# DCMMC/halo2-scaffold

Measured on AMD Instinct MI355X. Metric: create_proof() wall-clock + MSM G1-adds/s at k=20 standard_plonk, 1/2/4/8 GPU, higher is better.
Workload: dtype u32 (254-bit Montgomery integers as 9 x 29-bit limbs, 64-bit multiply-accumulate); 1 GPU; standard_plonk hot-path replay k=20: 11 MSM(2^20) + 6 iNTT(2^20) + 6 coset-NTT(2^21) + 1 coset-iNTT(2^21); k=20, scalar_distribution=uniform, msm_window_bits=17, msm_windows=15, msm_buckets=65536, parallelism=single-gpu, deployment=one process, one GPU, combine=none (single GPU)

## Files before the change

### halo2-scaffold_amd/csrc/h2mi_msm.hip

```cpp

#include <algorithm>
#include <map>
#include <type_traits>
#include <vector>

#include "g1.cuh"
#include "g1_29.cuh"
#include "g1_29_quad.cuh"
#include "h2mi_internal.h"
#include "scan.cuh"

namespace h2 {

constexpr uint32_t S0_MAX = 128;
constexpr uint32_t S1 = 8;
constexpr uint32_t FG_NARROW = 8;
constexpr uint32_t FG_WIDE = 2;
constexpr size_t SHIFT_MIN_N = 4096;
constexpr uint32_t HOT_MIN = 64;
constexpr uint32_t HOT_MIN_WIDE = 8;

constexpr uint32_t ACCUM_RESIDENT_CHUNKS = 256 * 2 * 256;
__host__ __device__ inline uint32_t accum_rounds(uint32_t entries) {
  const uint32_t per_round = S0_MAX * ACCUM_RESIDENT_CHUNKS;
// ... 20 lines not shown
  hipError_t wait(hipStream_t s) const { return hipStreamWaitEvent(s, ev, 0); }
  hipError_t wait_if_pending(hipStream_t s) const { return pending ? wait(s) : hipSuccess; }
  hipError_t wait_if_ever(hipStream_t s) const { return ever ? wait(s) : hipSuccess; }
};

struct Slot {
  uint32_t* vals[2] = {nullptr, nullptr};
  uint8_t* bkeys = nullptr;
  uint32_t* bincnt = nullptr;
  uint32_t* binbase = nullptr;
  uint32_t* binseg = nullptr;
  uint32_t* tile_live = nullptr;
  uint32_t* off = nullptr;
  uint32_t* s0_dev = nullptr;
  uint32_t* np[2] = {nullptr, nullptr};
  uint32_t* toff[2] = {nullptr, nullptr};
  uint8_t* part[2] = {nullptr, nullptr};
  uint8_t* dense = nullptr;
  uint8_t *dense2 = nullptr, *vsum = nullptr;
  uint32_t* tseg[2] = {nullptr, nullptr};
  uint8_t* rc = nullptr;
  uint8_t* g = nullptr;
  uint64_t* stats = nullptr;
  fe* shift = nullptr;
  Stage input_ready;
  Stage head, accum, tail;
  hipStream_t last_stream = nullptr;
  bool tail_deferred = false;
  void* d_out = nullptr;
  uint32_t tasks1 = 0;
  uint8_t* sdig = nullptr;
  uint8_t* spart = nullptr;
  uint32_t* scnt = nullptr;
  bool small_deferred = false;
  uint32_t small_n = 0;

  hipError_t create_events() {
    for (Stage* st : {&input_ready, &head, &accum, &tail})
      if (hipError_t e = st->create()) return e;
    return hipSuccess;
  }
  void destroy_events() {
    for (Stage* st : {&input_ready, &head, &accum, &tail}) st->destroy();
  }
  void clear_pending() { tail.pending = accum.pending = head.pending = false; }
  hipError_t reduction_launched(hipStream_t t) {
    const hipError_t e = tail.record(t);
    if (e == hipSuccess) tail_deferred = small_deferred = false;
    return e;
  }
};
constexpr int NSLOT = 8;

struct Bases {
  int dev = 0;
  size_t n = 0;
  size_t stride = 0;
  bool has_sum = false;
  uint32_t c = 0, W = 0, nb = 0, logNl = 0, logNh = 0;
  uint32_t seg_log = 0;
  uint8_t* table = nullptr;
  uint8_t* host_stage = nullptr;
  uint32_t lb = 0, nbins = 0;
  Slot slot[NSLOT];
  int nslot = NSLOT;
  int next_slot = 0, last_slot = 0;
  uint32_t max_tasks0 = 0, max_tasks1 = 0;
  bool small = false;
  uint32_t sc = 0, sW = 0, slanes = 0, sr = 0, sG = 0;
  uint8_t* stable = nullptr;
  uint32_t since_join = 0;
  bool last_small = false;
};

static std::map<uint64_t, Bases*> g_bases;
struct AdHoc {
  size_t n;
  uint64_t fp[2];
  uint64_t handle;
  uint64_t last_use;
};
static std::vector<AdHoc> g_adhoc;
static uint64_t g_adhoc_clock = 0, g_adhoc_builds = 0;
constexpr size_t ADHOC_MAX = 4;
static bool g_canonical = false;
constexpr size_t SMALL_STREAM_N = (size_t)1 << 13;
constexpr uint32_t SMALL_STREAM_AFTER = 4;
static uint64_t g_next_handle = 1;

__global__ void __launch_bounds__(256) k_msm_table_first(const uint8_t* bases, uint8_t* table0, size_t n) {
  size_t i = (size_t)blockIdx.x * blockDim.x + threadIdx.x;
  if (i >= n) return;
  affine p = affine_load(bases + i * 64);
  if (!affine_is_identity(p)) {
    f29 x, y;
    affine_to_f29(p, x, y);
    f29_pack(x, p.x.v);
    f29_pack(y, p.y.v);
  }
  affine_store(table0 + i * 64, p);
}
__global__ void __launch_bounds__(256) k_msm_table_next(const uint8_t* prev, uint8_t* next, size_t n, uint32_t c) {
  size_t i = (size_t)blockIdx.x * blockDim.x + threadIdx.x;
  if (i >= n) return;
  affine p = affine_load(prev + i * 64);
  if (affine_is_identity(p)) {
    affine_store(next + i * 64, p);
    return;
  }
  xyzz29 acc = xyzz29_dbl_affine(f29_unpack(p.x.v), f29_unpack(p.y.v));
  for (uint32_t k = 1; k < c; k++) acc = xyzz29_dbl(acc);
  f29 x, y;
  xyzz29_to_affine(acc, x, y);
  affine q;
  f29_pack(x, q.x.v);
  f29_pack(y, q.y.v);
  affine_store(next + i * 64, q);
}

__global__ void __launch_bounds__(64) k_msm_table_sum_point(const uint8_t* sum_jac, uint8_t* table, size_t stride, size_t n, uint32_t W, uint32_t c) {
  const uint32_t w = threadIdx.x;
  if (w >= W) return;
  const xyzz29 b = xyzz29_from_jac(jac_load(sum_jac));
  affine out;
  out.x = fe_zero();
  out.y = fe_zero();
  if (!xyzz29_is_identity(b)) {
    f29 x, y;
    xyzz29_to_affine(b, x, y);
    if (w) {
      xyzz29 acc = xyzz29_dbl_affine(x, y);
      for (uint32_t k = 1; k < c * w; k++) acc = xyzz29_dbl(acc);
      xyzz29_to_affine(acc, x, y);
    }
    f29_pack(x, out.x.v);
    f29_pack(y, out.y.v);
  }
  affine_store(table + ((size_t)w * stride + n) * 64, out);
}
__global__ void __launch_bounds__(256) k_msm_fill_one(fe* out, size_t n) {
  size_t i = (size_t)blockIdx.x * blockDim.x + threadIdx.x;
  if (i < n) fe_store(&out[i], fe_one<FrP>());
}

constexpr uint32_t P1_TS = 768;
constexpr uint32_t NBINS_MAX = 512;
constexpr uint32_t WIDE_MIN_C = 18, WIDE_MAX_C = 20, MAT_LOG = 16;
constexpr uint32_t WIDE_BIN_BITS = 9;
template <bool WIDE>
__device__ __forceinline__ uint32_t bin_of(uint32_t bucket, uint32_t lb) { return WIDE ? (bucket & ((1u << WIDE_BIN_BITS) - 1)) : (bucket >> lb); }
template <bool WIDE>
__device__ __forceinline__ uint32_t key_of(uint32_t bucket, uint32_t mask) { return WIDE ? (bucket >> WIDE_BIN_BITS) : (bucket & mask); }
constexpr uint32_t P2_THREADS = 512, P2_PER = 16, P2_CH = P2_THREADS * P2_PER;

template <uint32_t CT, class F>
__device__ __forceinline__ void for_each_digit(const fe& s, uint32_t c_rt, uint32_t W_rt, F&& f) {
  const uint32_t c = CT ? CT : c_rt;
  const uint32_t W = CT ? (255 + CT - 1) / CT : W_rt;
  uint32_t carry = 0;
  const uint32_t half = 1u << (c - 1);
#pragma unroll
  for (uint32_t w = 0; w < W; w++) {
    uint32_t bit = w * c;
    uint32_t limb = bit >> 5, sh = bit & 31;
    uint32_t raw = 0;
    if (limb < 8) {
      uint64_t two = s.v[limb];
      if (limb + 1 < 8) two |= (uint64_t)s.v[limb + 1] << 32;
      raw = (uint32_t)(two >> sh) & ((1u << c) - 1);
    }
    uint32_t d = raw + carry;
    uint32_t mag = d, neg = 0;
    carry = 0;
    if (d > half) {
      mag = (1u << c) - d;
      neg = 1;
      carry = 1;
    }
    if (mag) f(w, mag - 1, neg);
  }
}


__device__ __forceinline__ void msm_pick_shift_body(const fe* scalars, size_t n, fe* shift_out) {
  __shared__ fe smp[64];
  const uint32_t lane = threadIdx.x;
  size_t idx = (n / 64) * lane + n / 128;
  if (idx >= n) idx = n - 1;
  const fe v = fe_load(&scalars[idx]);
  smp[lane] = v;
  __syncthreads();
  uint32_t same = 0;
  for (uint32_t j = 0; j < 64; j++) same += fe_eq(v, smp[j]) ? 1u : 0u;
  const uint64_t winners = __ballot(same >= 40);
  if (lane == 0) fe_store(shift_out, winners ? smp[__ffsll((unsigned long long)winners) - 1] : fe_zero());
}
__global__ void __launch_bounds__(64) k_msm_pick_shift(const fe* scalars, size_t n, fe* shift_out) { msm_pick_shift_body(scalars, n, shift_out); }
__device__ __forceinline__ fe msm_scalar(const fe* scalars, size_t i, size_t n, const fe* shift) {
  fe x;
  if (!shift) {
    x = fe_load(&scalars[i]);
  } else {
    const fe v = fe_load(shift);
    x = i < n ? fe_sub<FrP>(fe_load(&scalars[i]), v) : v;
  }
  if (fe_is_zero(x)) return x;
  f29 c = f29_zero();
  c.v[0] = 32;
  fe o;
  f29_pack(f29_reduce_canonical<Fr29>(f29_mul<Fr29>(f29_unpack(x.v), c)), o.v);
  return o;
}

template <uint32_t CT>
__device__ __forceinline__ void msm_bin_count_body(const fe* scalars, size_t n, const fe* shift, uint32_t c, uint32_t W, uint32_t lb, uint32_t nbins,
                                                   uint32_t ntiles, uint32_t* cnt_out, uint32_t* tile_live) {
  __shared__ uint32_t cnt[NBINS_MAX];
  __shared__ uint32_t any_live;
  const uint32_t tid = threadIdx.x;
  if (tid < NBINS_MAX) cnt[tid] = 0;
  if (tid == 0) any_live = 0;
  __syncthreads();
  size_t i = (size_t)blockIdx.x * P1_TS + tid;
  if (i < n + (shift ? 1 : 0)) {
    fe s = msm_scalar(scalars, i, n, shift);
    if (!fe_is_zero(s)) {
      any_live = 1;
      for_each_digit<CT>(s, c, W, [&](uint32_t, uint32_t bucket, uint32_t) { atomicAdd(&cnt[bin_of<(CT >= WIDE_MIN_C)>(bucket, lb)], 1u); });
    }
  }
  __syncthreads();
  if (tid == 0) tile_live[blockIdx.x] = any_live;
  if (tid < nbins) cnt_out[(size_t)tid * ntiles + blockIdx.x] = cnt[tid];
  if (blockIdx.x == 0 && tid == 0) cnt_out[(size_t)nbins * ntiles] = 0;
}
template <uint32_t CT>
__global__ void __launch_bounds__(P1_TS) k_msm_bin_count(const fe* scalars, size_t n, const fe* shift, uint32_t c, uint32_t W, uint32_t lb,
                                                         uint32_t nbins, uint32_t ntiles, uint32_t* cnt_out, uint32_t* tile_live) {
  msm_bin_count_body<CT>(scalars, n, shift, c, W, lb, nbins, ntiles, cnt_out, tile_live);
}

extern __shared__ uint4 h2_msm_smem[];

template <uint32_t CT>
__device__ __forceinline__ void msm_bin_scatter_body(const fe* scalars, size_t n, const fe* shift, size_t n_reg, uint32_t c, uint32_t W, uint32_t lb,
                                                     uint32_t nbins, uint32_t ntiles, const uint32_t* base, uint32_t* vals_out, void* keys_out_,
                                                     const uint32_t* tile_live) {
  constexpr bool WIDE = CT >= WIDE_MIN_C;
  if (!tile_live[blockIdx.x]) return;
  __shared__ uint32_t cnt[NBINS_MAX], lstart[NBINS_MAX + 1], wsum[NBINS_MAX / 64];
  uint32_t* stage_val = reinterpret_cast<uint32_t*>(h2_msm_smem);
  uint16_t* stage_key = reinterpret_cast<uint16_t*>(stage_val + P1_TS * W);
  const uint32_t tid = threadIdx.x, lane = tid & 63, wave = tid >> 6, tile = blockIdx.x;
  uint32_t gb = 0;
  if (tid < NBINS_MAX) {
    cnt[tid] = 0;
    gb = tid < nbins ? base[(size_t)tid * ntiles + tile] : 0;
  }
  __syncthreads();
  size_t i = (size_t)tile * P1_TS + tid;
  fe s;
  const bool live = i < n + (shift ? 1 : 0);
  constexpr uint32_t WK = CT ? (255 + CT - 1) / CT : 1;
  uint32_t ent[WK], rk[WK];
#pragma unroll
  for (uint32_t w = 0; w < WK; w++) ent[w] = 0xFFFFFFFFu;
  bool live_nz = false;
  if (live) {
    s = msm_scalar(scalars, i, n, shift);
    live_nz = !fe_is_zero(s);
  }
  if (live_nz) {
    for_each_digit<CT>(s, c, W, [&](uint32_t w, uint32_t bucket, uint32_t neg) {
      uint32_t r = atomicAdd(&cnt[bin_of<WIDE>(bucket, lb)], 1u);
      if (CT) {
        ent[w] = bucket | (neg << 31);
        rk[w] = r;
      }
    });
  }
  __syncthreads();
  uint32_t v = 0, inc = 0;
  if (tid < NBINS_MAX) {
    v = cnt[tid];
    inc = wave_incl_scan(v);
    if (lane == 63) wsum[wave] = inc;
  }
  __syncthreads();
  if (tid < NBINS_MAX) {
    uint32_t add = 0;
    for (uint32_t j = 0; j < wave; j++) add += wsum[j];
    lstart[tid] = add + inc - v;
    cnt[tid] = add + inc - v;
    if (tid == NBINS_MAX - 1) lstart[NBINS_MAX] = add + inc;
  }
  __syncthreads();
  const uint32_t mask = (1u << lb) - 1;
  if (CT) {
#pragma unroll
    for (uint32_t w = 0; w < WK; w++)
      if (ent[w] != 0xFFFFFFFFu) {
        const uint32_t bucket = ent[w] & 0x7FFFFFFFu;
        const uint32_t pos = lstart[bin_of<WIDE>(bucket, lb)] + rk[w];
        stage_val[pos] = (ent[w] & 0x80000000u) | (uint32_t)((size_t)w * n_reg + i);
        stage_key[pos] = (uint16_t)(WIDE ? key_of<true>(bucket, mask) : bucket);
      }
  } else if (live_nz) {
    for_each_digit<CT>(s, c, W, [&](uint32_t w, uint32_t bucket, uint32_t neg) {
      uint32_t pos = atomicAdd(&cnt[bucket >> lb], 1u);
      stage_val[pos] = (neg << 31) | (uint32_t)((size_t)w * n_reg + i);
      stage_key[pos] = (uint16_t)bucket;
    });
  }
  __syncthreads();
  if (tid < NBINS_MAX) cnt[tid] = gb - lstart[tid];
  __syncthreads();
  const uint32_t total = lstart[NBINS_MAX];
  if (WIDE) {
    uint16_t* keys_out = reinterpret_cast<uint16_t*>(keys_out_);
    for (uint32_t p = tid; p < total; p += P1_TS) {
      uint32_t lo = 0, hi = NBINS_MAX;
      while (hi - lo > 1) {
        const uint32_t mid = (lo + hi) >> 1;
        if (lstart[mid] <= p) lo = mid;
        else hi = mid;
      }
      const uint32_t dst = p + cnt[lo];
      vals_out[dst] = stage_val[p];
      keys_out[dst] = stage_key[p];
    }
  } else {
    uint8_t* keys_out = reinterpret_cast<uint8_t*>(keys_out_);
    for (uint32_t p = tid; p < total; p += P1_TS) {
      const uint32_t key = stage_key[p];
      const uint32_t dst = p + cnt[key >> lb];
      vals_out[dst] = stage_val[p];
      keys_out[dst] = (uint8_t)(key & mask);
    }
  }
}
template <uint32_t CT>
__global__ void __launch_bounds__(P1_TS) k_msm_bin_scatter(const fe* scalars, size_t n, const fe* shift, size_t n_reg, uint32_t c, uint32_t W,
                                                           uint32_t lb, uint32_t nbins, uint32_t ntiles, const uint32_t* base, uint32_t* vals_out,
                                                           void* keys_out_, const uint32_t* tile_live) {
  msm_bin_scatter_body<CT>(scalars, n, shift, n_reg, c, W, lb, nbins, ntiles, base, vals_out, keys_out_, tile_live);
}

constexpr uint32_t NQ_MAX = 128;
__device__ __forceinline__ void msm_bin_sort_body(const uint8_t* keys_in, const uint32_t* vals_in, const uint32_t* base, uint32_t ntiles, uint32_t nbins,
                                                  uint32_t lb, uint32_t s0_fixed, uint32_t nb, uint32_t* vals_out, uint32_t* off, uint32_t* np0,
                                                  uint32_t* np1, uint32_t* s0_out) {
  __shared__ uint32_t wh[P2_THREADS / 64][NQ_MAX];
  __shared__ uint32_t run[NQ_MAX], ccnt[NQ_MAX], cstart[NQ_MAX], carry64;
  __shared__ uint32_t stage[P2_CH];
  __shared__ uint8_t stage_q[P2_CH];
  const uint32_t tid = threadIdx.x, wave = tid >> 6, bin = blockIdx.x;
  const uint32_t start = base[(size_t)bin * ntiles], end = base[(size_t)(bin + 1) * ntiles];
  const uint32_t nq = 1u << lb;
  const uint32_t entries = base[(size_t)nbins * ntiles];
  const uint32_t s0 = s0_fixed ? s0_fixed : accum_chunk_len(entries);
  for (uint32_t j = tid; j < (P2_THREADS / 64) * NQ_MAX; j += P2_THREADS) (&wh[0][0])[j] = 0;
  __syncthreads();
  for (uint32_t j = (start & ~15u) + tid * 16; j < end; j += P2_THREADS * 16) {
    const uint4 kk = *reinterpret_cast<const uint4*>(keys_in + j);
    const uint32_t w4[4] = {kk.x, kk.y, kk.z, kk.w};
#pragma unroll
    for (uint32_t t = 0; t < 16; t++) {
      const uint32_t idx = j + t;
      if (idx >= start && idx < end) atomicAdd(&wh[wave][(w4[t >> 2] >> (8 * (t & 3))) & (NQ_MAX - 1)], 1u);
    }
  }
  __syncthreads();
  uint32_t tot = 0, inc = 0;
  if (tid < NQ_MAX) {
#pragma unroll
    for (uint32_t w = 0; w < P2_THREADS / 64; w++) tot += wh[w][tid];
    inc = wave_incl_scan(tot);
    if (tid == 63) carry64 = inc;
  }
  __syncthreads();
  if (tid < NQ_MAX) {
    const uint32_t ex = inc - tot + (tid >= 64 ? carry64 : 0);
    run[tid] = start + ex;
    ccnt[tid] = 0;
    if (tid < nq) {
      const uint32_t b = (bin << lb) + tid;
      const uint32_t o = start + ex;
      off[b] = o;
      uint32_t f0 = tot ? 1u + (o + tot - 1) / s0 - o / s0 : 0u;
      np0[b] = f0;
      np1[b] = (f0 + S1 - 1) / S1;
    }
    if (bin == 0 && tid == 0) {
      off[nb] = entries;
      np0[nb] = 0;
      np1[nb] = 0;
      *s0_out = s0;
    }
  }
  __syncthreads();
  for (uint32_t cs = start; cs < end; cs += P2_CH) {
    const uint32_t m = min(P2_CH, end - cs);
    uint32_t q[P2_PER], v[P2_PER], r[P2_PER];
#pragma unroll
    for (uint32_t k = 0; k < P2_PER; k++) {
      const uint32_t p = k * P2_THREADS + tid;
      if (p < m) {
        q[k] = keys_in[cs + p] & (NQ_MAX - 1);
        v[k] = vals_in[cs + p];
      }
    }
#pragma unroll
    for (uint32_t k = 0; k < P2_PER; k++)
      if (k * P2_THREADS + tid < m) r[k] = atomicAdd(&ccnt[q[k]], 1u);
    __syncthreads();
    uint32_t cn = 0, cinc = 0;
    if (tid < NQ_MAX) {
      cn = ccnt[tid];
      cinc = wave_incl_scan(cn);
      if (tid == 63) carry64 = cinc;
    }
    __syncthreads();
    if (tid < NQ_MAX) cstart[tid] = cinc - cn + (tid >= 64 ? carry64 : 0);
    __syncthreads();
#pragma unroll
    for (uint32_t k = 0; k < P2_PER; k++)
      if (k * P2_THREADS + tid < m) {
        const uint32_t pos = cstart[q[k]] + r[k];
        stage[pos] = v[k];
        stage_q[pos] = (uint8_t)q[k];
      }
    __syncthreads();
    for (uint32_t p = tid; p < m; p += P2_THREADS) {
      const uint32_t qq = stage_q[p];
      vals_out[run[qq] + (p - cstart[qq])] = stage[p];
    }
    __syncthreads();
    if (tid < NQ_MAX) {
      run[tid] += ccnt[tid];
      ccnt[tid] = 0;
    }
    __syncthreads();
  }
}
__global__ void __launch_bounds__(P2_THREADS) k_msm_bin_sort(const uint8_t* keys_in, const uint32_t* vals_in, const uint32_t* base, uint32_t ntiles,
                                                             uint32_t nbins, uint32_t lb, uint32_t s0_fixed, uint32_t nb, uint32_t* vals_out,
                                                             uint32_t* off, uint32_t* np0, uint32_t* np1, uint32_t* s0_out) {
  msm_bin_sort_body(keys_in, vals_in, base, ntiles, nbins, lb, s0_fixed, nb, vals_out, off, np0, np1, s0_out);
}

constexpr uint32_t NQW = 1024, P2W_PER = 12, P2W_CH = P2_THREADS * P2W_PER;
__device__ __forceinline__ void block_excl_scan_1024(const uint32_t* in, uint32_t* out, uint32_t* wtot ) {
  const uint32_t tid = threadIdx.x, lane = tid & 63, wave = tid >> 6;
  const uint32_t a = in[2 * tid], b = in[2 * tid + 1];
  const uint32_t inc = wave_incl_scan(a + b);
  if (lane == 63) wtot[wave] = inc;
  __syncthreads();
  uint32_t add = 0;
  for (uint32_t w = 0; w < wave; w++) add += wtot[w];
  const uint32_t ex = add + inc - (a + b);
  __syncthreads();
  out[2 * tid] = ex;
  out[2 * tid + 1] = ex + a;
}
__global__ void __launch_bounds__(P2_THREADS) k_msm_bin_sort_wide(const uint16_t* keys_in, const uint32_t* vals_in, const uint32_t* base,
                                                                  uint32_t ntiles, uint32_t nbins, uint32_t lb, uint32_t s0_fixed, uint32_t nb,
                                                                  uint32_t* vals_out, uint32_t* off, uint32_t* np0, uint32_t* np1, uint32_t* s0_out) {
  __shared__ uint32_t hist[NQW], run[NQW], ccnt[NQW], cstart[NQW], wtot[P2_THREADS / 64];
  __shared__ uint32_t stage[P2W_CH];
  __shared__ uint16_t stage_q[P2W_CH];
  const uint32_t tid = threadIdx.x, bin = blockIdx.x;
  const uint32_t start = base[(size_t)bin * ntiles], end = base[(size_t)(bin + 1) * ntiles];
  const uint32_t nq = 1u << lb;
  const uint32_t entries = base[(size_t)nbins * ntiles];
  const uint32_t s0 = s0_fixed ? s0_fixed : accum_chunk_len(entries);
  for (uint32_t j = tid; j < NQW; j += P2_THREADS) {
    hist[j] = 0;
    ccnt[j] = 0;
  }
  __syncthreads();
  for (uint32_t j = (start & ~7u) + tid * 8; j < end; j += P2_THREADS * 8) {
    const uint4 kk = *reinterpret_cast<const uint4*>(keys_in + j);
    const uint32_t w4[4] = {kk.x, kk.y, kk.z, kk.w};
#pragma unroll
    for (uint32_t t = 0; t < 8; t++) {
      const uint32_t idx = j + t;
      if (idx >= start && idx < end) atomicAdd(&hist[(w4[t >> 1] >> (16 * (t & 1))) & (NQW - 1)], 1u);
    }
  }
  __syncthreads();
  block_excl_scan_1024(hist, cstart, wtot);
  __syncthreads();
  for (uint32_t q = tid; q < NQW; q += P2_THREADS) {
    const uint32_t ex = cstart[q], tot = hist[q];
    run[q] = start + ex;
    if (q < nq) {
      const uint32_t b = (bin << lb) + q;
      const uint32_t o = start + ex;
      off[b] = o;
      const uint32_t f0 = tot ? 1u + (o + tot - 1) / s0 - o / s0 : 0u;
      np0[b] = f0;
      np1[b] = (f0 + S1 - 1) / S1;
    }
  }
  if (bin == 0 && tid == 0) {
    off[nb] = entries;
    np0[nb] = 0;
    np1[nb] = 0;
    *s0_out = s0;
  }
  __syncthreads();
  for (uint32_t cs = start; cs < end; cs += P2W_CH) {
    const uint32_t m = min(P2W_CH, end - cs);
    uint32_t q[P2W_PER], v[P2W_PER], r[P2W_PER];
#pragma unroll
    for (uint32_t k = 0; k < P2W_PER; k++) {
      const uint32_t p = k * P2_THREADS + tid;
      if (p < m) {
        q[k] = keys_in[cs + p] & (NQW - 1);
        v[k] = vals_in[cs + p];
      }
    }
#pragma unroll
    for (uint32_t k = 0; k < P2W_PER; k++)
      if (k * P2_THREADS + tid < m) r[k] = atomicAdd(&ccnt[q[k]], 1u);
    __syncthreads();
    block_excl_scan_1024(ccnt, cstart, wtot);
    __syncthreads();
#pragma unroll
    for (uint32_t k = 0; k < P2W_PER; k++)
      if (k * P2_THREADS + tid < m) {
        const uint32_t pos = cstart[q[k]] + r[k];
        stage[pos] = v[k];
        stage_q[pos] = (uint16_t)q[k];
      }
    __syncthreads();
    for (uint32_t p = tid; p < m; p += P2_THREADS) {
      const uint32_t qq = stage_q[p];
      vals_out[run[qq] + (p - cstart[qq])] = stage[p];
    }
    __syncthreads();
    for (uint32_t qi = tid; qi < NQW; qi += P2_THREADS) {
      run[qi] += ccnt[qi];
      ccnt[qi] = 0;
    }
    __syncthreads();
  }
}

constexpr uint32_t PART_BYTES = 144;
__device__ __forceinline__ xyzz29 part_load(const uint8_t* p) {
  const uint4* q = reinterpret_cast<const uint4*>(p);
  uint32_t w[36];
#pragma unroll
  for (int i = 0; i < 9; i++) {
    uint4 v = q[i];
    w[4 * i] = v.x; w[4 * i + 1] = v.y; w[4 * i + 2] = v.z; w[4 * i + 3] = v.w;
  }
  xyzz29 r;
#pragma unroll
  for (int i = 0; i < 9; i++) { r.x.v[i] = w[i]; r.y.v[i] = w[9 + i]; r.zz.v[i] = w[18 + i]; r.zzz.v[i] = w[27 + i]; }
  return r;
}
__device__ __forceinline__ void part_store(uint8_t* p, const xyzz29& a) {
  uint32_t w[36];
#pragma unroll
  for (int i = 0; i < 9; i++) { w[i] = a.x.v[i]; w[9 + i] = a.y.v[i]; w[18 + i] = a.zz.v[i]; w[27 + i] = a.zzz.v[i]; }
  uint4* q = reinterpret_cast<uint4*>(p);
#pragma unroll
  for (int i = 0; i < 9; i++) q[i] = make_uint4(w[4 * i], w[4 * i + 1], w[4 * i + 2], w[4 * i + 3]);
}

__device__ __forceinline__ uint32_t find_bucket(const uint32_t* toff, uint32_t nb, uint32_t t) {
  uint32_t lo = 0, hi = nb;
  while (hi - lo > 1) {
    uint32_t mid = (lo + hi) >> 1;
    if (toff[mid] <= t) lo = mid;
    else hi = mid;
  }
  return lo;
}

typedef affine tab_entry;
__device__ __forceinline__ tab_entry tab_load(const uint8_t* table, uint32_t i) { return affine_load(table + (size_t)i * 64); }
__device__ __forceinline__ bool tab_is_identity(const tab_entry& p) { return affine_is_identity(p); }
__device__ __forceinline__ f29 tab_x(const tab_entry& p) { return f29_unpack(p.x.v); }
__device__ __forceinline__ f29 tab_y(const tab_entry& p) { return f29_unpack(p.y.v); }

__device__ __forceinline__ void msm_accum_body(const uint32_t* entries, const uint32_t* off, const uint32_t* toff, uint32_t nb, const uint32_t* s0_dev,
                                               const uint8_t* table, uint8_t* part) {
  const uint32_t t = blockIdx.x * blockDim.x + threadIdx.x;
  const uint32_t total = off[nb];
  const uint32_t s0 = *s0_dev;
  if ((uint64_t)t * s0 >= total) return;
  const uint32_t start = t * s0;
  const uint32_t end = min(start + s0, total);
  uint32_t b = find_bucket(off, nb, start);
  uint32_t pidx = toff[b] + (t - off[b] / s0);
  uint32_t bend = off[b + 1];
  xyzz29 acc = xyzz29_identity();
  uint32_t e = entries[start];
  tab_entry nxt = tab_load(table, e & 0x7fffffffu);
  uint32_t nneg = e >> 31;
  for (uint32_t k = start; k < end; k++) {
    if (k == bend) {
      part_store(part + (size_t)pidx * PART_BYTES, acc);
      pidx++;
      acc = xyzz29_identity();
      do {
        b++;
        bend = off[b + 1];
      } while (bend == k);
    }
    tab_entry p = nxt;
    uint32_t neg = nneg;
    if (k + 1 < end) {
      e = entries[k + 1];
      nxt = tab_load(table, e & 0x7fffffffu);
      nneg = e >> 31;
    }
    if (tab_is_identity(p)) continue;
    f29 x2 = tab_x(p);
    f29 y2 = tab_y(p);
    if (neg) y2 = f29_sub(f29_zero(), y2, Fq29::K2);
    xyzz29_madd(acc, x2, y2);
  }
  part_store(part + (size_t)pidx * PART_BYTES, acc);
}
__global__ void __launch_bounds__(256) k_msm_accum(const uint32_t* entries, const uint32_t* off, const uint32_t* toff, uint32_t nb,
                                                    const uint32_t* s0_dev, const uint8_t* table, uint8_t* part) {
  msm_accum_body(entries, off, toff, nb, s0_dev, table, part);
}

constexpr size_t ACCUM_LDS = 56000;

constexpr uint32_t HEAD_BATCH = 4;
struct HeadDesc {
  const fe* scalars;
  fe* shift;
  uint32_t *bincnt, *tile_live, *binseg, *binbase, *vals0, *vals1, *off, *np0, *np1, *toff0, *toff1, *s0_dev;
  void* bkeys;
  uint8_t* part0;
};
struct HeadBatch {
  HeadDesc d[HEAD_BATCH];
};
__global__ void __launch_bounds__(64) k_msm_pick_shift_b(const HeadBatch hb, size_t n) {
  const HeadDesc& d = hb.d[blockIdx.y];
  msm_pick_shift_body(d.scalars, n, d.shift);
}
template <uint32_t CT>
__global__ void __launch_bounds__(P1_TS) k_msm_bin_count_b(const HeadBatch hb, size_t n, uint32_t c, uint32_t W, uint32_t lb, uint32_t nbins,
                                                           uint32_t ntiles) {
  const HeadDesc& d = hb.d[blockIdx.y];
  msm_bin_count_body<CT>(d.scalars, n, d.shift, c, W, lb, nbins, ntiles, d.bincnt, d.tile_live);
}
template <uint32_t CT>
__global__ void __launch_bounds__(P1_TS) k_msm_bin_scatter_b(const HeadBatch hb, size_t n, size_t n_reg, uint32_t c, uint32_t W, uint32_t lb,
                                                             uint32_t nbins, uint32_t ntiles) {
  const HeadDesc& d = hb.d[blockIdx.y];
  msm_bin_scatter_body<CT>(d.scalars, n, d.shift, n_reg, c, W, lb, nbins, ntiles, d.binbase, d.vals0, d.bkeys, d.tile_live);
}
__global__ void __launch_bounds__(P2_THREADS) k_msm_bin_sort_b(const HeadBatch hb, uint32_t ntiles, uint32_t nbins, uint32_t lb, uint32_t s0_fixed,
                                                               uint32_t nb) {
  const HeadDesc& d = hb.d[blockIdx.y];
  msm_bin_sort_body((const uint8_t*)d.bkeys, d.vals0, d.binbase, ntiles, nbins, lb, s0_fixed, nb, d.vals1, d.off, d.np0, d.np1, d.s0_dev);
}
__global__ void __launch_bounds__(256) k_msm_accum_b(const HeadBatch hb, uint32_t nb, const uint8_t* table) {
  const HeadDesc& d = hb.d[blockIdx.y];
  msm_accum_body(d.vals1, d.off, d.toff0, nb, d.s0_dev, table, d.part0);
}
__global__ void __launch_bounds__(1024) k_scan_segsum_bins_b(const HeadBatch hb, uint32_t m) {
  const HeadDesc& d = hb.d[blockIdx.y];
  scan_segsum_body<SCAN_SEG_BINS>(d.bincnt, m, d.binseg);
}
__global__ void __launch_bounds__(1024) k_scan_seg_bins_b(const HeadBatch hb, uint32_t m) {
  const HeadDesc& d = hb.d[blockIdx.y];
  scan_seg_body<SCAN_SEG_BINS>(d.bincnt, d.binbase, m, d.binseg);
}
__global__ void __launch_bounds__(1024) k_scan_seg_tasks_b(const HeadBatch hb, uint32_t m) {
  const HeadDesc& d = hb.d[blockIdx.z];
  scan_seg_body<SCAN_SEG_TASKS>(blockIdx.y ? d.np1 : d.np0, blockIdx.y ? d.toff1 : d.toff0, m, nullptr);
}

constexpr uint32_t TAIL_BATCH = 8;
struct TailDesc {
  const uint8_t* part0;
  const uint32_t *toff0, *np0, *toff1, *np1, *off;
  uint8_t *part1, *dense, *rc, *g, *out;
  uint64_t* stats;
  uint32_t nb, logNh, logNl, canonical;
  const uint8_t* mat;
  uint8_t *dense2, *vsum;
  uint32_t seg_log;
  uint32_t hot_min;
  uint32_t no_fold;
};
struct TailBatch {
  TailDesc d[TAIL_BATCH];
};

constexpr uint32_t TAIL_THREADS = 512;

template <bool QUAD>
__global__ void __launch_bounds__(256) k_msm_fold(const TailBatch tb) {
  const TailDesc& d = tb.d[blockIdx.y];
  if (d.no_fold) return;
  const uint32_t nb = d.nb;
  const uint32_t *toff_out = d.toff1, *toff_in = d.toff0, *np_in = d.np0;
  const uint32_t t = (blockIdx.x * blockDim.x + threadIdx.x) >> (QUAD ? 2 : 0);
  if (t >= toff_out[nb]) return;
  uint32_t b = find_bucket(toff_out, nb, t);
  uint32_t j = t - toff_out[b];
  const uint32_t m = np_in[b], np = toff_out[b + 1] - toff_out[b];
  const uint32_t q = m / np, r = m - q * np;
  uint32_t start = toff_in[b] + j * q + min(j, r);
  uint32_t len = q + (j < r ? 1u : 0u);
  xyzz29 acc = part_load(d.part0 + (size_t)start * PART_BYTES);
  for (uint32_t k = 1; k < len; k++) {
    xyzz29 p = part_load(d.part0 + (size_t)(start + k) * PART_BYTES);
    if (QUAD) acc = xyzz29_add_quad(acc, p);
    else xyzz29_add(acc, p);
  }
  if (!QUAD || (threadIdx.x & 3u) == 0) part_store(d.part1 + (size_t)t * PART_BYTES, acc);
}

__device__ __forceinline__ xyzz29 shfl_down_xyzz(const xyzz29& a, uint32_t delta) {
  xyzz29 r;
#pragma unroll
  for (int i = 0; i < 9; i++) {
    r.x.v[i] = __shfl_down(a.x.v[i], delta);
    r.y.v[i] = __shfl_down(a.y.v[i], delta);
    r.zz.v[i] = __shfl_down(a.zz.v[i], delta);
    r.zzz.v[i] = __shfl_down(a.zzz.v[i], delta);
  }
  return r;
}
__device__ __forceinline__ void msm_finish_hot_body(const TailDesc& d, uint32_t bx);
template <bool QUAD, uint32_t FG>
__global__ void __launch_bounds__(256) k_msm_finish(const TailBatch tb, uint32_t hot_blocks) {
  const TailDesc& d = tb.d[blockIdx.y];
  if (blockIdx.x < hot_blocks) {
    msm_finish_hot_body(d, blockIdx.x);
    return;
  }
  const uint32_t bx = blockIdx.x - hot_blocks;
  const uint32_t nb = d.nb;
  constexpr uint32_t LW = QUAD ? 2 : 0;
  const uint32_t worker = (bx * blockDim.x + threadIdx.x) >> LW;
  const uint32_t b = worker / FG, l = worker % FG;
  if ((bx * blockDim.x >> LW) / FG >= nb) return;
  xyzz29 acc = xyzz29_identity();
  bool hot = false;
  if (b < nb) {
    uint32_t cnt = d.np1[b], s = d.toff1[b];
    hot = cnt > d.hot_min;
    if (hot) cnt = 0;
    for (uint32_t k = l; k < cnt; k += FG) {
      xyzz29 p = part_load(d.part1 + (size_t)(s + k) * PART_BYTES);
      if (QUAD) acc = xyzz29_add_quad(acc, p);
      else xyzz29_add(acc, p);
    }
  }
  for (uint32_t dd = FG / 2; dd > 0; dd >>= 1) {
    xyzz29 o = shfl_down_xyzz(acc, dd << LW);
    if (l < dd) {
      if (QUAD) acc = xyzz29_add_quad(acc, o);
      else xyzz29_add(acc, o);
    }
  }
  if (b < nb && !hot && l == 0 && (!QUAD || (threadIdx.x & 3u) == 0)) part_store(d.dense + (size_t)b * PART_BYTES, acc);
}

__device__ __forceinline__ void block_tree_sum(xyzz29* lds, uint32_t count_pow2) {
  const uint32_t quad = threadIdx.x >> 2, nquads = blockDim.x >> 2;
  for (uint32_t s = count_pow2 >> 1; s > 0; s >>= 1) {
    for (uint32_t g = quad; g < s; g += nquads) {
      xyzz29 r = xyzz29_add_quad(lds[g], lds[g + s]);
      if ((threadIdx.x & 3u) == 0) lds[g] = r;
    }
    __syncthreads();
  }
}

__device__ __forceinline__ void msm_finish_hot_body(const TailDesc& d, uint32_t bx) {
  __shared__ uint32_t hot_list[256], nhot;
  const uint32_t tid = threadIdx.x, quad = tid >> 2;
  const uint32_t b = bx * 256 + tid;
  if (tid == 0) nhot = 0;
  __syncthreads();
  if (b < d.nb && d.np1[b] > d.hot_min) hot_list[atomicAdd(&nhot, 1u)] = b;
  __syncthreads();
  const uint32_t n_hot = nhot;
  xyzz29* lds = reinterpret_cast<xyzz29*>(h2_msm_smem);
  for (uint32_t h = 0; h < n_hot; h++) {
    const uint32_t hb = hot_list[h];
    const uint32_t cnt = d.np1[hb], s = d.toff1[hb];
    xyzz29 acc = xyzz29_identity();
    for (uint32_t k = quad; k < cnt; k += 64) acc = xyzz29_add_quad(acc, part_load(d.part1 + (size_t)(s + k) * PART_BYTES));
    if ((tid & 3u) == 0) lds[quad] = acc;
    __syncthreads();
    block_tree_sum(lds, 64);
    if (tid == 0) part_store(d.dense + (size_t)hb * PART_BYTES, lds[0]);
    __syncthreads();
  }
}

__global__ void __launch_bounds__(256) k_msm_seg(const TailBatch tb) {
  const TailDesc& d = tb.d[blockIdx.y];
  if (!d.seg_log) return;
  const uint32_t L = 1u << d.seg_log, s = (blockIdx.x * blockDim.x + threadIdx.x) >> 2;
  if (s >= (d.nb >> d.seg_log)) return;
  const uint32_t lb = MAT_LOG + d.seg_log - WIDE_BIN_BITS;
  xyzz29 T = xyzz29_identity(), V = xyzz29_identity();
  for (uint32_t j = 0; j < L; j++) {
    const uint32_t b = s * L + j, bp = ((b & ((1u << WIDE_BIN_BITS) - 1)) << lb) | (b >> WIDE_BIN_BITS);
    V = xyzz29_add_quad(V, T);
    T = xyzz29_add_quad(T, part_load(d.dense + (size_t)bp * PART_BYTES));
  }
  if ((threadIdx.x & 3u) == 0) {
    part_store(d.dense2 + (size_t)s * PART_BYTES, T);
// ... 524 lines not shown
    work[j].S->tail_deferred = true;
    work[j].S->small_deferred = small;
    g_deferred.push_back(work[j]);
  }
  if (g_deferred.size() >= (size_t)std::max(1, work[0].B->nslot / 2)) return flush_tails();
  return H2MI_OK;
}

static bool pipelined(hipStream_t s, bool inorder) { return !inorder && s == ctx().stream && ctx().tail_stream && !getenv("H2MI_MSM_NO_PIPELINE"); }

static int msm_small(Bases* B, const void* const* d_scalars, size_t m, size_t n, void* d_out, hipStream_t s, bool inorder, bool batch) {
  const bool deferred = pipelined(s, inorder);
  Deferred work[HEAD_BATCH];
  SmallHeadBatch hb;
  for (size_t j = 0; j < m; j++) {
    Slot* slot;
    int rc = acquire_slot(B, slot);
    if (rc) return rc;
    Slot& S = *slot;
    if (S.tail.ever && (S.tail.pending || (!deferred && !batch) || S.last_stream != s)) H2_HIP(S.tail.wait(s));
    H2_HIP(S.head.wait_if_pending(s));
    H2_HIP(S.accum.wait_if_pending(s));
    S.clear_pending();
    S.last_stream = s;
    S.d_out = (char*)d_out + 96 * j;
    S.small_n = (uint32_t)n;
    hb.scalars[j] = (const fe*)d_scalars[j];
    hb.dig[j] = S.sdig;
    work[j] = {B, &S};
  }
  if (batch) {
    pad_descs(hb.scalars, m);
    pad_descs(hb.dig, m);
    H2_LAUNCH("k_msm_small_digits", k_msm_small_digits_b, dim3(ceil_div_u32(n, 64), (uint32_t)m), 64, 0, s, hb, (uint32_t)n, (uint32_t)B->n, B->sc, B->sW);
  } else {
    H2_LAUNCH("k_msm_small_digits", k_msm_small_digits, ceil_div_u32(n, 64), 64, 0, s, hb.scalars[0], (uint32_t)n, (uint32_t)B->n, B->sc, B->sW, hb.dig[0]);
  }
  if (deferred)
    for (size_t j = 0; j < m; j++) H2_HIP(work[j].S->accum.record(s));
  return reduce_or_defer(work, m, true, deferred, s);
}

static int msm_general(Bases* B, const void* const* d_scalars, size_t m, size_t n, void* d_out, hipStream_t s, bool inorder, bool batch) {
  const uint32_t nb = B->nb, W = B->W, mm = (uint32_t)m;
  const bool shifted = B->has_sum && n == B->n;
  const size_t n_eff = n + (shifted ? 1 : 0);
  const uint32_t total = (uint32_t)(n_eff * W), ntiles = ceil_div_u32(n_eff, P1_TS);
  uint32_t s0_fixed = chunk_override();
  while (s0_fixed && s0_fixed < S0_MAX && ((uint64_t)total + s0_fixed - 1) / s0_fixed + nb > B->max_tasks0) s0_fixed++;
  if (s0_fixed && ((uint64_t)total + s0_fixed - 1) / s0_fixed + nb > B->max_tasks0) return H2MI_ERANGE;
  if ((size_t)P1_TS * W * 6 > (size_t)SCATTER_LDS_MAX) return H2MI_ERANGE;
  const uint32_t chunks0 = s0_fixed ? (uint32_t)(((uint64_t)total + s0_fixed - 1) / s0_fixed) : std::min(accum_rounds(total) * ACCUM_RESIDENT_CHUNKS, total);
  const uint32_t tasks0 = chunks0 + nb;
  const bool deferred = pipelined(s, inorder);
  const bool staged = deferred || batch;
  const hipStream_t hs = deferred ? ctx().head_stream : s, as = !deferred ? s : batch ? hs : ctx().accum_stream;
  Deferred work[HEAD_BATCH];
  HeadBatch hb;
  for (size_t j = 0; j < m; j++) {
    Slot* slot;
    int rc = acquire_slot(B, slot);
    if (rc) return rc;
    Slot& S = *slot;
    if (staged) {
      H2_HIP(S.head.wait_if_pending(s));
      if (S.tail.pending && S.last_stream != s) H2_HIP(S.tail.wait(s));
    } else {
      H2_HIP(S.head.wait_if_ever(s));
      H2_HIP(S.accum.wait_if_ever(s));
      H2_HIP(S.tail.wait_if_ever(s));
    }
    S.last_stream = s;
    S.d_out = (char*)d_out + 96 * j;
    S.tasks1 = tasks0 / S1 + nb;
    work[j] = {B, &S};
    if (batch) {
      HeadDesc& d = hb.d[j];
      d.scalars = (const fe*)d_scalars[j];
      d.shift = shifted ? S.shift : nullptr;
      d.bincnt = S.bincnt; d.tile_live = S.tile_live; d.binseg = S.binseg; d.binbase = S.binbase;
      d.vals0 = S.vals[0]; d.vals1 = S.vals[1]; d.bkeys = S.bkeys;
      d.off = S.off; d.np0 = S.np[0]; d.np1 = S.np[1]; d.toff0 = S.toff[0]; d.toff1 = S.toff[1]; d.s0_dev = S.s0_dev;
      d.part0 = S.part[0];
    }
  }
  Slot& S0 = *work[0].S;
  if (batch) pad_descs(hb.d, m);
  int rc = batch ? launch_level1_b(B, hb, mm, n, shifted, ntiles, s) : launch_level1(B, S0, (const fe*)d_scalars[0], n, shifted, ntiles, s);
  if (rc) return rc;
  if (hs != s) {
    H2_HIP(S0.input_ready.record(s));
    H2_HIP(S0.input_ready.wait(hs));
  }
  for (size_t j = 0; j < m; j++) {
    Slot& S = *work[j].S;
    if (staged) {
      H2_HIP(S.accum.wait_if_pending(hs));
      H2_HIP(S.tail.wait_if_pending(hs));
    }
    S.clear_pending();
  }
  rc = batch ? launch_level2_b(B, hb, mm, ntiles, s0_fixed, hs) : launch_level2(B, S0, ntiles, s0_fixed, hs);
  if (rc) return rc;
  if (staged) {
    for (size_t j = 0; j < m; j++) H2_HIP(work[j].S->head.record(hs));
    if (as != hs) H2_HIP(work[m - 1].S->head.wait(as));
  }
  if (batch) {
    H2_LAUNCH("k_msm_accum", k_msm_accum_b, dim3(ceil_div_u32(chunks0, 256), mm), 256, ACCUM_LDS, as, hb, nb, (const uint8_t*)B->table);
  } else {
    H2_LAUNCH("k_msm_accum", k_msm_accum, ceil_div_u32(chunks0, 256), 256, ACCUM_LDS, as, (const uint32_t*)S0.vals[1], (const uint32_t*)S0.off,
              (const uint32_t*)S0.toff[0], nb, (const uint32_t*)S0.s0_dev, (const uint8_t*)B->table, S0.part[0]);
  }
  if (staged)
    for (size_t j = 0; j < m; j++) H2_HIP(work[j].S->accum.record(as));
  return reduce_or_defer(work, m, false, deferred, s);
}

static bool take_small(const Bases* B, bool general) {
  return B->small && !general && !(B->n > SMALL_STREAM_N && B->since_join >= SMALL_STREAM_AFTER);
}
constexpr size_t HEAD_BATCH_MAX_N = (size_t)1 << 17;
static int msm_group(Bases* B, const void* const* d_scalars, size_t m, size_t n, void* d_out, hipStream_t s, bool inorder, bool general, bool batch) {
  B->last_small = take_small(B, general);
  B->since_join += (uint32_t)m;
  return B->last_small ? msm_small(B, d_scalars, m, n, d_out, s, inorder, batch) : msm_general(B, d_scalars, m, n, d_out, s, inorder, batch);
}
static int msm_dev(Bases* B, const void* d_scalars, size_t n, void* d_out, hipStream_t s, bool inorder = false, bool general = false) {
  return msm_group(B, &d_scalars, 1, n, d_out, s, inorder, general, false);
}

#define H2_ALLOC(ptr, bytes)                                   \
  do {                                                         \
    hipError_t e_ = hipMalloc((void**)&(ptr), (bytes));        \
    if (e_ != hipSuccess) {                                    \
      note_hip_error(e_, __FILE__, __LINE__);                  \
      free_bases(B);                                           \
      return e_ == hipErrorOutOfMemory ? H2MI_ENOMEM : H2MI_EHIP; \
    }                                                          \
  } while (0)

static int register_dev(const void* d_bases, size_t n, uint64_t* handle_out, hipStream_t s, bool allow_small = true) {
  if (n == 0 || n > ((size_t)1 << 26)) return H2MI_ERANGE;
  Bases* B = new Bases();
  B->n = n;
  B->dev = ctx().cur;
  B->stride = n + 1;
  B->c = pick_window(n);
  B->W = (255 + B->c - 1) / B->c;
  B->nb = 1u << (B->c - 1);
  B->seg_log = B->c - 1 > MAT_LOG ? B->c - 1 - MAT_LOG : 0;
  B->logNl = (B->c - 1 - B->seg_log + 1) / 2;
  B->logNh = (B->c - 1 - B->seg_log) - B->logNl;
  if ((uint64_t)B->stride * B->W >= (1ull << 31)) { delete B; return H2MI_ERANGE; }
  const size_t nW = B->stride * B->W;
  B->max_tasks0 = std::min(accum_rounds((uint32_t)nW) * ACCUM_RESIDENT_CHUNKS, (uint32_t)nW) + B->nb + 1;
  B->max_tasks1 = B->max_tasks0 / S1 + B->nb;
  H2_ALLOC(B->table, nW * 64);
  B->lb = B->c - 1 > 9 ? B->c - 1 - 9 : 0;
  B->nbins = B->nb >> B->lb;
  const size_t ntiles_max = (B->stride + P1_TS - 1) / P1_TS;
  const size_t bin_cells = (size_t)B->nbins * ntiles_max + 1;
  if (bin_cells >= ((size_t)1 << 31)) { free_bases(B); return H2MI_ERANGE; }
  if ((B->nbins & 3u) || B->nb < 4 || (B->nb > SCAN_SEG_TASKS && !B->seg_log) || B->nbins > NBINS_MAX || (1u << B->lb) > NQW) { free_bases(B); return H2MI_ERANGE; }
  B->nslot = n > ((size_t)1 << 17) ? 4 : NSLOT;
  for (int si_ = 0; si_ < B->nslot; si_++) {
    Slot& S = B->slot[si_];
    for (int i = 0; i < 2; i++) H2_ALLOC(S.vals[i], nW * 4);
    H2_ALLOC(S.bkeys, nW * (B->seg_log ? 2 : 1) + 16);
    H2_ALLOC(S.bincnt, bin_cells * 4);
    H2_ALLOC(S.binbase, bin_cells * 4);
    H2_ALLOC(S.binseg, (bin_cells / SCAN_SEG_BINS + 2) * 4);
    H2_ALLOC(S.tile_live, (ntiles_max + 1) * 4);
    H2_ALLOC(S.off, (size_t)(B->nb + 1) * 4);
    H2_ALLOC(S.s0_dev, 4);
    for (int i = 0; i < 2; i++) {
      H2_ALLOC(S.np[i], (size_t)(B->nb + 1) * 4);
      H2_ALLOC(S.toff[i], (size_t)(B->nb + 1) * 4);
    }
    H2_ALLOC(S.dense, (size_t)B->nb * PART_BYTES);
    if (B->seg_log) {
      H2_ALLOC(S.dense2, ((size_t)1 << MAT_LOG) * PART_BYTES);
      H2_ALLOC(S.vsum, ((size_t)1 << MAT_LOG) * PART_BYTES);
      for (int i = 0; i < 2; i++) H2_ALLOC(S.tseg[i], (size_t)(B->nb / SCAN_SEG_BINS + 2) * 4);
    }
    H2_ALLOC(S.part[0], (size_t)B->max_tasks0 * PART_BYTES);
    H2_ALLOC(S.part[1], (size_t)B->max_tasks1 * PART_BYTES);
    H2_ALLOC(S.rc, (size_t)((2u << B->logNh) + (1u << B->logNl)) * PART_BYTES);
    H2_ALLOC(S.g, (size_t)64 * PART_BYTES);
    H2_ALLOC(S.stats, 64);
    H2_ALLOC(S.shift, 32);
    if (S.create_events() != hipSuccess) {
      free_bases(B);
      return H2MI_EHIP;
    }
  }
  {
    const bool prof_ = prof_on("k_msm_table_first");
    if (prof_) prof_begin("k_msm_table_first", s);
    hipLaunchKernelGGL(k_msm_table_first, dim3(ceil_div_u32(n, 256)), dim3(256), 0, s, (const uint8_t*)d_bases, B->table, n);
    if (prof_) prof_end(s);
  }
  for (uint32_t w = 1; w < B->W; w++) {
    const bool prof_ = prof_on("k_msm_table_next");
    if (prof_) prof_begin("k_msm_table_next", s);
    hipLaunchKernelGGL(k_msm_table_next, dim3(ceil_div_u32(n, 256)), dim3(256), 0, s, (const uint8_t*)(B->table + (size_t)(w - 1) * B->stride * 64),
                       B->table + (size_t)w * B->stride * 64, n, B->c);
    if (prof_) prof_end(s);
  }
  if (allow_small && small_geometry(n, &B->sc, &B->slanes, &B->sr)) {
    B->sW = (255 + B->sc - 1) / B->sc;
    B->sG = ceil_div_u32((uint64_t)n * B->sW, (uint64_t)B->slanes * B->sr);
    const uint32_t NBs = 1u << (B->sc - 1);
    const size_t plane = (size_t)B->sW * n;
    bool fits = hipMalloc((void**)&B->stable, (size_t)NBs * plane * 64) == hipSuccess;
    for (int si_ = 0; fits && si_ < B->nslot; si_++) {
      Slot& S = B->slot[si_];
      fits = hipMalloc((void**)&S.sdig, plane) == hipSuccess && hipMalloc((void**)&S.spart, (size_t)B->sG * PART_BYTES) == hipSuccess &&
             hipMalloc((void**)&S.scnt, (size_t)(B->sG + 1) * 4) == hipSuccess;
      if (fits && hipMemsetAsync(S.scnt, 0, (size_t)(B->sG + 1) * 4, s) != hipSuccess) { free_bases(B); return H2MI_EHIP; }
    }
    if (!fits) {
      (void)hipGetLastError();
      H2_IGNORE(hipStreamSynchronize(s));
      for (int si_ = 0; si_ < B->nslot; si_++) {
        Slot& S = B->slot[si_];
        if (S.sdig) H2_IGNORE(hipFree(S.sdig));
        if (S.spart) H2_IGNORE(hipFree(S.spart));
        if (S.scnt) H2_IGNORE(hipFree(S.scnt));
        S.sdig = nullptr; S.spart = nullptr; S.scnt = nullptr;
      }
      if (B->stable) H2_IGNORE(hipFree(B->stable));
      B->stable = nullptr;
    }
    if (fits) {
    if (hipMemcpyAsync(B->stable, B->table, n * 64, hipMemcpyDeviceToDevice, s) != hipSuccess) { free_bases(B); return H2MI_EHIP; }
    for (uint32_t w = 1; w < B->sW; w++)
      hipLaunchKernelGGL(k_msm_table_next, dim3(ceil_div_u32(n, 64)), dim3(64), 0, s, (const uint8_t*)(B->stable + (size_t)(w - 1) * n * 64),
                         B->stable + (size_t)w * n * 64, n, B->sc);
    hipLaunchKernelGGL(k_msm_small_multiples, dim3(ceil_div_u32(plane, 64)), dim3(64), 0, s, B->stable, plane, NBs);
    B->small = true;
    }
  }
  for (uint32_t w = 0; w < B->W; w++)
    if (hipMemsetAsync(B->table + ((size_t)w * B->stride + n) * 64, 0, 64, s) != hipSuccess) { free_bases(B); return H2MI_EHIP; }
  if (hipGetLastError() != hipSuccess || hipStreamSynchronize(s) != hipSuccess) { free_bases(B); return H2MI_EHIP; }
  const uint64_t h = g_next_handle++;
  g_bases[h] = B;
  if (n >= SHIFT_MIN_N && !B->small) {
    fe* ones = nullptr;
    uint8_t* sum = nullptr;
    int rc = H2MI_OK;
    if (hipMalloc((void**)&ones, n * 32) != hipSuccess || hipMalloc((void**)&sum, 96) != hipSuccess) rc = H2MI_ENOMEM;
    if (!rc) {
      hipLaunchKernelGGL(k_msm_fill_one, dim3(ceil_div_u32(n, 256)), dim3(256), 0, s, ones, n);
      rc = msm_dev(B, ones, n, sum, s);
    }
    if (!rc) rc = msm_join_all(s);
    if (!rc) {
      hipLaunchKernelGGL(k_msm_table_sum_point, dim3(1), dim3(64), 0, s, (const uint8_t*)sum, B->table, B->stride, n, B->W, B->c);
      if (hipGetLastError() != hipSuccess || hipStreamSynchronize(s) != hipSuccess) rc = H2MI_EHIP;
    }
    H2_IGNORE(hipFree(ones));
    H2_IGNORE(hipFree(sum));
    if (rc) {
      H2_IGNORE(hipDeviceSynchronize());
      g_bases.erase(h);
      free_bases(B);
      return rc;
    }
    B->has_sum = true;
  }
  *handle_out = h;
  return H2MI_OK;
}

struct Shard {
  uint64_t handle = 0;
  size_t lo = 0, hi = 0;
  uint8_t* stage = nullptr;
  uint8_t* part = nullptr;
  hipEvent_t ready = nullptr;
};
constexpr uint32_t SHARD_RING = 16;
struct Sharded {
  size_t n = 0;
  std::vector<Shard> shard;
  uint8_t* gather = nullptr;
  uint32_t next = 0;
};
struct PendingFold {
  Sharded* sh;
  uint32_t ring;
  void* d_out;
};
static std::map<uint64_t, Sharded*> g_sharded;
static std::vector<PendingFold> g_pending_folds;

static const uint64_t G1_IDENTITY[12] = {0, 0, 0, 0, 0xd35d438dc58f0d9dULL, 0x0a78eb28f5c70b3dULL, 0x666ea36f7879462cULL, 0x0e0a77c19a07df2fULL, 0, 0, 0, 0};

static hipError_t copy_between(void* dst, int dst_dev, const void* src, int src_dev, size_t bytes, hipStream_t s) {
  const int pd = ctx().devs[(size_t)dst_dev].device, ps = ctx().devs[(size_t)src_dev].device;
  if (pd == ps) return hipMemcpyAsync(dst, src, bytes, hipMemcpyDeviceToDevice, s);
  return hipMemcpyPeerAsync(dst, pd, src, ps, bytes, s);
}

static int fold_sharded(hipStream_t s0) {
// ... 463 lines not shown
```

Before: 9.448 billion G1-adds/s.

## Tag last-in-bucket entries during sort to simplify MSM accumulation loop

The bin-sort kernels now set a LAST flag bit on the final entry of each bucket. The accumulation kernel uses that flag to close a bucket instead of comparing against off[] boundaries and re-walking bucket offsets. It also gathers table points as raw 16-byte vectors one step ahead, with a cheaper identity test, and adds a min-blocks hint of 3 to the accum kernels to raise occupancy. The price is one more bit stolen from the entry index, which lowers the maximum table size, and register pressure from the occupancy hint may cause spills.

Result: no change. 9.570 billion G1-adds/s (median of 6 runs) (+1.3%).

```diff
diff --git a/halo2-scaffold_amd/csrc/h2mi_msm.hip b/halo2-scaffold_amd/csrc/h2mi_msm.hip
--- a/halo2-scaffold_amd/csrc/h2mi_msm.hip
+++ b/halo2-scaffold_amd/csrc/h2mi_msm.hip
@@ -196,6 +196,7 @@
 template <bool WIDE>
 __device__ __forceinline__ uint32_t key_of(uint32_t bucket, uint32_t mask) { return WIDE ? (bucket >> WIDE_BIN_BITS) : (bucket & mask); }
 constexpr uint32_t P2_THREADS = 512, P2_PER = 16, P2_CH = P2_THREADS * P2_PER;
+constexpr uint32_t ENTRY_NEG = 1u << 31, ENTRY_LAST = 1u << 30, ENTRY_INDEX = ENTRY_LAST - 1;
 
 template <uint32_t CT, class F>
 __device__ __forceinline__ void for_each_digit(const fe& s, uint32_t c_rt, uint32_t W_rt, F&& f) {
@@ -395,7 +396,7 @@
                                                   uint32_t lb, uint32_t s0_fixed, uint32_t nb, uint32_t* vals_out, uint32_t* off, uint32_t* np0,
                                                   uint32_t* np1, uint32_t* s0_out) {
   __shared__ uint32_t wh[P2_THREADS / 64][NQ_MAX];
-  __shared__ uint32_t run[NQ_MAX], ccnt[NQ_MAX], cstart[NQ_MAX], carry64;
+  __shared__ uint32_t run[NQ_MAX], ccnt[NQ_MAX], cstart[NQ_MAX], last[NQ_MAX], carry64;
   __shared__ uint32_t stage[P2_CH];
   __shared__ uint8_t stage_q[P2_CH];
   const uint32_t tid = threadIdx.x, wave = tid >> 6, bin = blockIdx.x;
@@ -426,6 +427,7 @@
   if (tid < NQ_MAX) {
     const uint32_t ex = inc - tot + (tid >= 64 ? carry64 : 0);
     run[tid] = start + ex;
+    last[tid] = start + ex + tot - 1;
     ccnt[tid] = 0;
     if (tid < nq) {
       const uint32_t b = (bin << lb) + tid;
@@ -477,7 +479,8 @@
     __syncthreads();
     for (uint32_t p = tid; p < m; p += P2_THREADS) {
       const uint32_t qq = stage_q[p];
-      vals_out[run[qq] + (p - cstart[qq])] = stage[p];
+      const uint32_t dst = run[qq] + (p - cstart[qq]);
+      vals_out[dst] = stage[p] | (dst == last[qq] ? ENTRY_LAST : 0u);
     }
     __syncthreads();
     if (tid < NQ_MAX) {
@@ -538,6 +541,7 @@
   for (uint32_t q = tid; q < NQW; q += P2_THREADS) {
     const uint32_t ex = cstart[q], tot = hist[q];
     run[q] = start + ex;
+    hist[q] = start + ex + tot - 1;
     if (q < nq) {
       const uint32_t b = (bin << lb) + q;
       const uint32_t o = start + ex;
@@ -581,7 +585,8 @@
     __syncthreads();
     for (uint32_t p = tid; p < m; p += P2_THREADS) {
       const uint32_t qq = stage_q[p];
-      vals_out[run[qq] + (p - cstart[qq])] = stage[p];
+      const uint32_t dst = run[qq] + (p - cstart[qq]);
+      vals_out[dst] = stage[p] | (dst == hist[qq] ? ENTRY_LAST : 0u);
     }
     __syncthreads();
     for (uint32_t qi = tid; qi < NQW; qi += P2_THREADS) {
@@ -625,12 +630,38 @@
   return lo;
 }
 
-typedef affine tab_entry;
-__device__ __forceinline__ tab_entry tab_load(const uint8_t* table, uint32_t i) { return affine_load(table + (size_t)i * 64); }
-__device__ __forceinline__ bool tab_is_identity(const tab_entry& p) { return affine_is_identity(p); }
-__device__ __forceinline__ f29 tab_x(const tab_entry& p) { return f29_unpack(p.x.v); }
-__device__ __forceinline__ f29 tab_y(const tab_entry& p) { return f29_unpack(p.y.v); }
-
+typedef uint32_t u32x4 __attribute__((ext_vector_type(4)));
+struct tab_stage {
+  u32x4 q[4];
+};
+__device__ __forceinline__ void tab_gather(tab_stage& s, const uint8_t* table, uint32_t e) {
+  const u32x4* src = reinterpret_cast<const u32x4*>(table + (size_t)(e & ENTRY_INDEX) * 64);
+#pragma unroll
+  for (int i = 0; i < 4; i++) s.q[i] = src[i];
+}
+__device__ __forceinline__ bool tab_unpack(const tab_stage& s, f29& x2, f29& y2) {
+  const uint32_t xw[8] = {s.q[0].x, s.q[0].y, s.q[0].z, s.q[0].w, s.q[1].x, s.q[1].y, s.q[1].z, s.q[1].w};
+  const uint32_t yw[8] = {s.q[2].x, s.q[2].y, s.q[2].z, s.q[2].w, s.q[3].x, s.q[3].y, s.q[3].z, s.q[3].w};
+  uint32_t o = 0;
+#pragma unroll
+  for (int i = 0; i < 8; i++) o |= xw[i] | yw[i];
+  x2 = f29_unpack(xw);
+  y2 = f29_unpack(yw);
+  return o != 0;
+}
+
+__device__ __forceinline__ void accum_insert(xyzz29& acc, uint32_t& pidx, uint8_t* part, const tab_stage& cur, uint32_t e) {
+  f29 x2, y2;
+  if (tab_unpack(cur, x2, y2)) {
+    if (e & ENTRY_NEG) y2 = f29_sub(f29_zero(), y2, Fq29::K2);
+    xyzz29_madd(acc, x2, y2);
+  }
+  if (e & ENTRY_LAST) {
+    part_store(part + (size_t)pidx * PART_BYTES, acc);
+    pidx++;
+    acc = xyzz29_identity();
+  }
+}
 __device__ __forceinline__ void msm_accum_body(const uint32_t* entries, const uint32_t* off, const uint32_t* toff, uint32_t nb, const uint32_t* s0_dev,
                                                const uint8_t* table, uint8_t* part) {
   const uint32_t t = blockIdx.x * blockDim.x + threadIdx.x;
@@ -639,39 +670,29 @@
   if ((uint64_t)t * s0 >= total) return;
   const uint32_t start = t * s0;
   const uint32_t end = min(start + s0, total);
-  uint32_t b = find_bucket(off, nb, start);
+  const uint32_t b = find_bucket(off, nb, start);
   uint32_t pidx = toff[b] + (t - off[b] / s0);
-  uint32_t bend = off[b + 1];
   xyzz29 acc = xyzz29_identity();
-  uint32_t e = entries[start];
-  tab_entry nxt = tab_load(table, e & 0x7fffffffu);
-  uint32_t nneg = e >> 31;
-  for (uint32_t k = start; k < end; k++) {
-    if (k == bend) {
-      part_store(part + (size_t)pidx * PART_BYTES, acc);
-      pidx++;
-      acc = xyzz29_identity();
-      do {
-        b++;
-        bend = off[b + 1];
-      } while (bend == k);
-    }
-    tab_entry p = nxt;
-    uint32_t neg = nneg;
-    if (k + 1 < end) {
-      e = entries[k + 1];
-      nxt = tab_load(table, e & 0x7fffffffu);
-      nneg = e >> 31;
-    }
-    if (tab_is_identity(p)) continue;
-    f29 x2 = tab_x(p);
-    f29 y2 = tab_y(p);
-    if (neg) y2 = f29_sub(f29_zero(), y2, Fq29::K2);
-    xyzz29_madd(acc, x2, y2);
-  }
-  part_store(part + (size_t)pidx * PART_BYTES, acc);
-}
-__global__ void __launch_bounds__(256) k_msm_accum(const uint32_t* entries, const uint32_t* off, const uint32_t* toff, uint32_t nb,
+  tab_stage cur, nxt;
+  uint32_t k = start;
+  uint32_t ea = entries[k];
+  tab_gather(cur, table, ea);
+  uint32_t eb = k + 1 < end ? entries[k + 1] : 0u;
+  uint32_t closed;
+  do {
+    const bool more = k + 1 < end;
+    if (more) tab_gather(nxt, table, eb);
+    const uint32_t ec = k + 2 < end ? entries[k + 2] : 0u;
+    accum_insert(acc, pidx, part, cur, ea);
+    closed = ea & ENTRY_LAST;
+    if (more) cur = nxt;
+    ea = eb;
+    eb = ec;
+    k++;
+  } while (k < end);
+  if (!closed) part_store(part + (size_t)pidx * PART_BYTES, acc);
+}
+__global__ void __launch_bounds__(256, 3) k_msm_accum(const uint32_t* entries, const uint32_t* off, const uint32_t* toff, uint32_t nb,
                                                     const uint32_t* s0_dev, const uint8_t* table, uint8_t* part) {
   msm_accum_body(entries, off, toff, nb, s0_dev, table, part);
 }
@@ -710,7 +731,7 @@
   const HeadDesc& d = hb.d[blockIdx.y];
   msm_bin_sort_body((const uint8_t*)d.bkeys, d.vals0, d.binbase, ntiles, nbins, lb, s0_fixed, nb, d.vals1, d.off, d.np0, d.np1, d.s0_dev);
 }
-__global__ void __launch_bounds__(256) k_msm_accum_b(const HeadBatch hb, uint32_t nb, const uint8_t* table) {
+__global__ void __launch_bounds__(256, 3) k_msm_accum_b(const HeadBatch hb, uint32_t nb, const uint8_t* table) {
   const HeadDesc& d = hb.d[blockIdx.y];
   msm_accum_body(d.vals1, d.off, d.toff0, nb, d.s0_dev, table, d.part0);
 }
@@ -1541,7 +1562,7 @@
   B->seg_log = B->c - 1 > MAT_LOG ? B->c - 1 - MAT_LOG : 0;
   B->logNl = (B->c - 1 - B->seg_log + 1) / 2;
   B->logNh = (B->c - 1 - B->seg_log) - B->logNl;
-  if ((uint64_t)B->stride * B->W >= (1ull << 31)) { delete B; return H2MI_ERANGE; }
+  if ((uint64_t)B->stride * B->W > (uint64_t)ENTRY_INDEX) { delete B; return H2MI_ERANGE; }
   const size_t nW = B->stride * B->W;
   B->max_tasks0 = std::min(accum_rounds((uint32_t)nW) * ACCUM_RESIDENT_CHUNKS, (uint32_t)nW) + B->nb + 1;
   B->max_tasks1 = B->max_tasks0 / S1 + B->nb;
```
